# rpng/open_vins

Measured on AMD Instinct MI355X. Metric: MSCKF features/sec per EKF update (30-clone state), higher is better.
Workload: dtype f64; 1 GPU; BASELINE.json configs[2]: 2-camera radtan rig, 30-clone window, 2000 MSCKF features/update, N=248, D=208, online cam extrinsic+intrinsic calib + IMU intrinsics in the state, FEJ; features_total=2000, features_this_rank=2000, clones=30, cameras=2, state_dim=248, measurements_total=100362, parallelism=single GPU

## Files before the change

open_vins_amd/csrc/api_context.inc:

```
using namespace ovg;

static thread_local std::string g_err = "";
static int set_err(int code, const std::string &msg) {
  g_err = msg;
  return code;
}

#define HIPCHK(expr)                                                                                         \
  do {                                                                                                       \
    hipError_t _e = (expr);                                                                                  \
    if (_e != hipSuccess) {                                                                                  \
      return set_err(OVGPU_ERR_HIP, std::string(#expr) + " -> " + hipGetErrorString(_e) + " (" __FILE__ ":" + \
                                        std::to_string(__LINE__) + ")");                                     \
    }                                                                                                        \
  } while (0)

namespace {

template <class T>
struct PinBuf {
  T *p = nullptr;
  size_t cap = 0;
  hipError_t reserve(size_t n) {
    if (n <= cap) return hipSuccess;
// ... 20 lines not shown
    p = nullptr;
    cap = 0;
    hipError_t e = hipMalloc((void **)&p, std::max<size_t>(n, 1) * sizeof(T));
    if (e == hipSuccess) cap = n;
    return e;
  }
  hipError_t grow(size_t n, size_t keep) {
    if (n <= cap) return hipSuccess;
    T *q = nullptr;
    hipError_t e = hipMalloc((void **)&q, n * sizeof(T));
    if (e != hipSuccess) return e;
    if (p && keep > 0) e = hipMemcpy(q, p, std::min(keep, cap) * sizeof(T), hipMemcpyDeviceToDevice);
    if (p) (void)hipFree(p);
    p = q, cap = n;
    return e;
  }
  void release() {
    if (p) (void)hipFree(p);
    p = nullptr;
    cap = 0;
  }
};

struct EventPair {
  hipEvent_t a = nullptr, b = nullptr;
};

}

enum { CTRL_FLAGS = 1, CTRL_ROWS = 2, CTRL_COUNTER = 4, CTRL_PROG0 = 8, CTRL_PROG1 = 16, CTRL_INTS = 64, CHOL_PROG_STRIDE = 24 };

struct LoopComm;
struct UpSeg {
  void *dst;
  uint32_t off, bytes;
};
constexpr int UP_MAX_SEG = 28, UP_BLOCKS = 48;
struct UpBatch {
  UpSeg seg[UP_MAX_SEG];
  int n = 0;
};
__global__ void __launch_bounds__(256) k_upload_scatter(const unsigned char *__restrict__ arena, UpBatch b) {
  const UpSeg sg = b.seg[blockIdx.y];
  const unsigned char *src = arena + sg.off;
  unsigned char *dst = static_cast<unsigned char *>(sg.dst);
  const uint32_t nvec = ((reinterpret_cast<uintptr_t>(dst) & 15) == 0) ? sg.bytes >> 4 : 0;
  typedef unsigned int u32x4 __attribute__((ext_vector_type(4)));
  const u32x4 *s4 = reinterpret_cast<const u32x4 *>(src);
  u32x4 *d4 = reinterpret_cast<u32x4 *>(dst);
  for (uint32_t i = blockIdx.x * 256 + threadIdx.x; i < nvec; i += gridDim.x * 256) d4[i] = __builtin_nontemporal_load(s4 + i);
  for (uint32_t i = (nvec << 4) + blockIdx.x * 256 + threadIdx.x; i < sg.bytes; i += gridDim.x * 256) dst[i] = src[i];
}

struct ovgpu_ctx {
  int device = 0;
  hipStream_t stream = nullptr;
  ovgpu_options opts{};
  DevOptions dopt{};
  int lds_limit = 160 * 1024;
  int num_cu = 256;

  bool have_state = false;
  bool poses_only = false;
  int N = 0, C = 0, K = 0, D = 0, LD = 0;
  DevBuf<double> P, P0, clone_qp, clone_qp0, clone_fej, calib_qp, calib_qp0, intr, intr0;
  DevBuf<uint8_t> fisheye;
  DevBuf<int32_t> clone_cov, calib_cov, intr_cov, clone_col, calib_col, intr_col, col_cov;
  DevBuf<uint8_t> col_kind, col_sub;
  DevBuf<uint16_t> col_var;
  DevBuf<double> tab_clone, tab_cam, tab_cc;
  std::vector<int32_t> h_col_cov;
  struct HVar { int cov, size, kind, index; };
  std::vector<HVar> h_vars;
  std::vector<int32_t> h_clone_cov, h_calib_cov, h_intr_cov;
  DevBuf<double> prop_w, prop_in;
  DevBuf<int32_t> prop_ids;
  int L = 0;
  std::vector<int32_t> h_lm_rep;
  std::vector<int32_t> h_feat_lm;
  std::vector<int32_t> h_feat_rep;
  std::vector<int32_t> h_lm_cov, h_lm_col, h_lm_anchor;
  DevBuf<double> pFej, lm_val, lm_fej;
  DevBuf<int32_t> feat_lm, feat_lmcol, feat_lmcov, feat_anchor, lm_cov, lm_col, lm_anchor, lm_repd, lm_index;
  bool slam_rows = false;
  int trk_max = 0, trk_obs = 0;
  int trk_group_order = OVGPU_GROUPS_REFERENCE;
  std::vector<std::vector<int8_t>> trk_h_cams;
  DevBuf<int8_t> trk_order;
  DevBuf<int32_t> trk_count, trk_cam, trk_slot_in, trk_cam_in, trk_sel, trk_nvalid, trk_flag;
  DevBuf<double> trk_time, trk_clone_times, trk_aux;
  DevBuf<float> trk_uv, trk_uvn, trk_uv_in, trk_uvn_in;
  std::unordered_map<int64_t, int32_t> trk_slot_of;
  std::unordered_map<int64_t, int32_t> retri_slot_of;
  DevBuf<double> retri_sys[2], retri_pos, retri_uvd;
  DevBuf<int32_t> retri_int, marg_idx, seed_anchor;
  DevBuf<double> marg_out, seed_pA;
  DevBuf<float> retri_f;
  int retri_gen = 0;
  std::vector<int32_t> trk_free, trk_h_count;
  std::vector<int64_t> trk_h_id;
  DevBuf<double> Ppad, init_ws, dx_seq;
  DevBuf<int32_t> init_ctr, feat_slot;
  bool init_export = false;
  DevBuf<double> isx_arena, isx_save;
  DevBuf<int32_t> isx_cols;
  std::vector<int32_t> h_isx_cols;

  bool have_feats = false;
  bool tri_readable = false;
  bool given_tri = false;
  bool given_has_anchor = false;
  std::vector<int32_t> h_given_status;
  DevBuf<int32_t> given_status;
  int F = 0, M = 0, m_max = 0;
  int64_t rows_total = 0;
  DevBuf<int32_t> meas_offsets;
  DevBuf<uint16_t> meas_cc;
  DevBuf<float> uv, uvn;
  DevBuf<int64_t> row_off;
  DevBuf<double> pA, pG, chi2, chi2_thr;
  int layout_every_update = 0;
  int inst_cb = 0, inst_D = 0;
  DevBuf<int32_t> anchor_pre;
  DevBuf<int32_t> anchor, status, sys_order;
  DevBuf<double> feat_sigma, feat_mult;
  bool have_feat_sigma = false, have_feat_mult = false;
  DevBuf<double> chi2_table;
  int chi2_table_len = 0;
  std::vector<double> h_chi2_table;
  std::vector<int32_t> h_offsets;
  std::vector<int64_t> h_row_off;

  DevBuf<double> Hbig, gate_ws, Rws, Mt, Aaug, Yaug, dx;
  DevBuf<int32_t> flags;
  int W = 1;
  int64_t rows_per_node = 128;
  DevBuf<QrTreeNode> tree_nodes, tree_nodes2;
  int tree_G2 = 0;
  hipStream_t stream2 = nullptr;
  hipEvent_t ev_rows = nullptr;
  bool gram_il = true;
  bool gram_blocks_only = false;
  bool fuse_chol_inputs = true;
  hipEvent_t ev_fork = nullptr, ev_join = nullptr;
  DevBuf<int32_t> leaf_flags;
  int tree_overlap = -1;
  bool tree_nodes_overlap = false, tree_nodes2_overlap = false;
  DevBuf<int32_t> tree_flags;
  DevBuf<int32_t> tree_err;
  int tree_G = 0;
  bool tree_pipelined = true;
  int compress_gram = 1;
  DevBuf<double> gram_part, gram_G, gram_rho, Yaug2, Lw;
  double prior_pivot_tol = 1e-13;
  int last_route = OVGPU_COMPRESS_GRAM;
  bool whiten = true;
  bool gram_is_whitened = false;
  bool prior_on_side = false;
  int feat_variant = 0;
  int feat_nt_max = 0;
  bool featy_ok = false;
  int featy_skip = 0;
  int featy_grid = 0;
  size_t featy_lds = 0;
  DevBuf<double> fs_tq;
  DevBuf<int32_t> fs_inst;
  DevBuf<double> featyb_ws;
  int featy_big = 0;
  bool no_feat_kernel = false;
  bool raw_enable = true;
  int raw_work_const = 12;
  bool raw_veto = false;
  bool raw_one_region = false;
  bool raw_cols_ok = false;
  bool raw_tables_ok = false;
  int raw_j0 = 0;
  int raw_ncls = 0, raw_ntc[RAW_MAXCLS + 1] = {0}, raw_ld[RAW_MAXCLS + 1] = {0}, raw_rcol[RAW_MAXCLS + 1] = {0};
  int64_t raw_base[RAW_MAXCLS + 1] = {0}, raw_rows[RAW_MAXCLS + 1] = {0};
  std::vector<uint8_t> h_cls_of_clone;
  DevBuf<uint8_t> cls_of_clone;
  DevBuf<int32_t> raw_featbase, raw_dst;
  DevBuf<double> Hraw;
  DevBuf<gram::GramRegionWG> gram_wg;
  int gram_wg_n = 0, gram_wg_tiles = 0;
  gram::GramRegionSum raw_rs;
  bool last_stack_raw = false;
  DevBuf<int32_t> feat_counter, fs_minfo, fs_meas_feat, fs_pos;
  DevBuf<int32_t> fs_slots;
  std::vector<int32_t> h_order;
  std::vector<uint16_t> h_cc;
  DevBuf<double> fs_rows, fs_V, fs_z, fs_w;
  void *comm = nullptr;
  struct LoopComm *loop = nullptr;
  int comm_rank = 0, comm_world = 1;
  DevBuf<double> comm_buf;
  DevBuf<int32_t> chol_prog;
  DevBuf<int32_t> ctrl;
  unsigned ctrl_clean = 0;
  unsigned ctrl_pre = 0;
  DevBuf<double> chol_uinv;
  PinBuf<double> h_tri;
  int chol_slot = 0;
  bool no_chol_pipe = false;
  int tri_waves = 0;
  int feat_shape = 0;
  int feat_nta_max = 0;
  PinBuf<unsigned char> up_arena;
  PinBuf<unsigned char> down_arena;
  size_t up_off = 0, up_want = 8u << 20;
  UpBatch up_batch;
  const unsigned char *up_arena_dev = nullptr;
  bool up_kernel = true;
  UpBatch down_batch;
  unsigned char *down_arena_dev = nullptr;
  const double *chi2_table_dev = nullptr;
  int chi2_table_dev_len = 0;
  bool up_dirty = false;
  bool up_fallback = false;
  bool gram_fp32 = false;
  bool want_stack_f32 = false;
  bool stack_is_f32 = false;
  int stack_ldf = 0;
  DevBuf<float> Hbig32, gram32_part;
  DevBuf<int32_t> gram32_tiles;
  int gram32_ntm = 0, gram32_P = 0;
  int Lw_D = -1;
  DevBuf<long long> dbg_cycles;
  int tsqr_workers = 0;
  bool async_pending = false;
  bool last_update_tform = false;
  bool force_tsqr = false;
  int chol_spin_limit = 1 << 22;
  int chol_timeouts = 0;
  int mode_a_factor = 0;
  bool factor_from_gram = false;
  bool last_factor_from_gram = false;
  bool chol_timed_out = false;
  bool prior_pending = false;
  bool prior_overlap = true;
  const double *last_uinv = nullptr;
  const double *prior_uinv = nullptr;
  int layout_fpw = 8;
  bool unwhiten_blocked = true;
  bool pchol_blocked = true;
  bool speculative_prior = true;
  DevBuf<int32_t> gram_dropped, rows_used;
  int sys_grid = 1;
  int64_t gate_ws_stride = 0;
  bool sys_rows_global = false;
  DevBuf<double> sys_rows_ws;
  int m_lds_max = 0;
  size_t sys_lds_bytes = 0;
  int row_stride = 48;

  std::vector<EventPair> ev_compress, ev_update, ev_system;
  size_t ev_used = 0;
  bool timed_this_update = false;
  bool timing = true;
  int timing_period = 1;
  uint64_t timing_seq = 0;
};

template <class T>
static hipError_t remove_record(DevBuf<T> &a, DevBuf<T> &tmp, int n, int w, int idx, hipStream_t s) {
  const size_t tail = (size_t)(n - idx - 1) * w;
  if (tail == 0) return hipSuccess;
  hipError_t e = tmp.reserve(tail);
  if (e != hipSuccess) return e;
  e = hipMemcpyAsync(tmp.p, a.p + (size_t)(idx + 1) * w, tail * sizeof(T), hipMemcpyDeviceToDevice, s);
  if (e != hipSuccess) return e;
  return hipMemcpyAsync(a.p + (size_t)idx * w, tmp.p, tail * sizeof(T), hipMemcpyDeviceToDevice, s);
}

static hipError_t upload(void *dst, const void *src, size_t bytes, hipStream_t s) {
  if (bytes == 0) return hipSuccess;
  return hipMemcpyAsync(dst, src, bytes, hipMemcpyHostToDevice, s);
}

static hipError_t upload_flush(ovgpu_ctx *c);
static hipError_t upload_begin(ovgpu_ctx *c) {
  if (!c->up_dirty) c->up_off = 0;
  if (c->up_want > c->up_arena.cap) {
    if (c->up_dirty) {
      if (hipError_t ef = upload_flush(c); ef != hipSuccess) return ef;
      hipError_t e = hipStreamSynchronize(c->stream);
      if (e != hipSuccess) return e;
      c->up_dirty = false, c->up_fallback = false, c->up_off = 0;
    }
    if (hipError_t e = c->up_arena.reserve(c->up_want); e != hipSuccess) return e;
    void *dev = nullptr;
    c->up_arena_dev = hipHostGetDevicePointer(&dev, c->up_arena.p, 0) == hipSuccess ? static_cast<const unsigned char *>(dev) : nullptr;
  }
  return hipSuccess;
}
__global__ void __launch_bounds__(256) k_download_gather(unsigned char *__restrict__ arena, UpBatch b) {
  const UpSeg sg = b.seg[blockIdx.y];
  unsigned char *dst = arena + sg.off;
  const unsigned char *src = static_cast<const unsigned char *>(sg.dst);
  const uint32_t nvec = ((reinterpret_cast<uintptr_t>(src) & 15) == 0) ? sg.bytes >> 4 : 0;
  typedef unsigned int u32x4 __attribute__((ext_vector_type(4)));
  const u32x4 *s4 = reinterpret_cast<const u32x4 *>(src);
  u32x4 *d4 = reinterpret_cast<u32x4 *>(dst);
  for (uint32_t i = blockIdx.x * 256 + threadIdx.x; i < nvec; i += gridDim.x * 256) __builtin_nontemporal_store(s4[i], d4 + i);
  for (uint32_t i = (nvec << 4) + blockIdx.x * 256 + threadIdx.x; i < sg.bytes; i += gridDim.x * 256) dst[i] = src[i];
}
static hipError_t down_reserve(ovgpu_ctx *c, size_t bytes) {
// ... 199 lines not shown
```

open_vins_amd/csrc/api_pipeline.inc:

```
static int enqueue_triangulate(ovgpu_ctx *c, const double *seed_pA = nullptr, const int32_t *seed_anchor = nullptr) {
  if (c->F == 0) return OVGPU_OK;
  TriParams p;
  p.seed_pA = seed_pA, p.seed_anchor = seed_anchor, p.anchor_pre = c->anchor_pre.p;
  p.F = c->F, p.C = c->C, p.K = c->K;
  p.meas_offsets = c->meas_offsets.p, p.meas_cc = c->meas_cc.p, p.uvn = c->uvn.p, p.tab_cc = c->tab_cc.p;
  p.p_FinA = c->pA.p, p.p_FinG = c->pG.p, p.anchor_meas = c->anchor.p, p.status = c->status.p;
  p.opt = c->dopt;
  const size_t lds = (size_t)c->K * c->C * 12 * sizeof(double);
  int wpb = c->tri_waves;
  if (wpb == 0) {
    wpb = 4;
    const int room = c->num_cu - 6;
    for (int w = 4; w <= 8 && room > 0; w *= 2) {
      const int blocks = (c->F + w - 1) / w;
      if (blocks <= room) {
        if (4 * blocks >= 3 * room) wpb = w;
        break;
      }
    }
  }
  hipLaunchKernelGGL(k_triangulate, dim3((c->F + wpb - 1) / wpb), dim3(64 * wpb), lds, c->stream, p);
  HIPCHK(hipGetLastError());
  return OVGPU_OK;
}
// ... 392 lines not shown
  double sigma2 = -1.0;
  const int32_t *pred = nullptr;
  double *dx = nullptr;
  bool keep_flags = false;
};

struct CholSource {
  int src = chol::CH_SRC_MATRIX;
  const TformParams *t = nullptr;
};
static int enqueue_chol_carry(ovgpu_ctx *c, const EkfParams &p, hipStream_t s, double *Lt, const CholSource &from = CholSource());

static int enqueue_ekf(ovgpu_ctx *c, const EkfJob &job = EkfJob()) {
  {
    const int rdp = drop_pending_prior(c);
    if (rdp != OVGPU_OK) return rdp;
  }
  c->last_update_tform = false;
  EkfParams p;
  const bool tri = job.R == nullptr;
  p.N = c->N, p.D = tri ? c->D : job.rows, p.DC = c->D, p.LD = c->LD, p.LA = p.D + c->N + 1, p.tri = tri ? 1 : 0, p.pred = job.pred;
  p.R = tri ? c->Rws.p : job.R, p.col_cov = job.col_cov ? job.col_cov : c->col_cov.p, p.P = c->P.p, p.Mt = c->Mt.p, p.A = c->Aaug.p, p.Y = c->Yaug.p;
  p.dx = job.dx ? job.dx : c->dx.p, p.flags = c->flags.p;
  p.sigma2 = job.sigma2 >= 0.0 ? job.sigma2 : c->dopt.sigma_pix_sq;
  hipStream_t s = c->stream;
  if (!job.keep_flags) HIPCHK(ctrl_zero(c, CTRL_FLAGS, c->flags.p, 4 * sizeof(int32_t), s));
  const int tm = (p.D + 15) / 16, tn = (p.N + 15) / 16;
  hipLaunchKernelGGL(k_ekf_mt, dim3((tm * tn + 3) / 4), dim3(256), 0, s, p);
  hipLaunchKernelGGL(k_ekf_s, dim3((tm * tm + 3) / 4), dim3(256), 0, s, p);
  {
    const int rcc = enqueue_chol_carry(c, p, s, nullptr);
    if (rcc != OVGPU_OK) return rcc;
  }
  hipLaunchKernelGGL(k_ekf_dx, dim3((p.N + 255) / 256), dim3(256), 0, s, p);
  hipLaunchKernelGGL(k_ekf_pupdate, dim3((tn * tn + 3) / 4), dim3(256), 0, s, p);
  const int n = std::max(c->C, c->K);
  hipLaunchKernelGGL(k_boxplus, dim3((n + 255) / 256), dim3(256), 0, s, c->C, c->K, p.dx, c->clone_cov.p, c->calib_cov.p, c->intr_cov.p,
                     c->clone_qp.p, c->calib_qp.p, c->intr.p, job.pred);
  HIPCHK(hipGetLastError());
  return launch_build_tables(c);
}

static bool chol_pipe_usable(const ovgpu_ctx *c, int D) { return !c->no_chol_pipe && D <= 16 * chol::CH_TMAX && D >= 1; }
static int enqueue_chol_carry(ovgpu_ctx *c, const EkfParams &p, hipStream_t s, double *Lt, const CholSource &from) {
  if (chol_pipe_usable(c, p.D)) {
    HIPCHK(c->chol_prog.reserve(CHOL_PROG_STRIDE + 16));
    HIPCHK(c->chol_uinv.reserve((size_t)2 * 16 * 256));
    const int slot = (c->chol_slot++) & 1;
    chol::CholParams q;
    q.D = p.D, q.LA = p.LA, q.A = p.A, q.Y = p.Y, q.Lt = Lt, q.flags = p.flags, q.diag0 = p.diag0, q.pivot_tol = p.pivot_tol, q.pred = p.pred;
    q.prog = c->chol_prog.p + CHOL_PROG_STRIDE * slot, q.uinv = c->chol_uinv.p + (size_t)slot * 16 * 256, q.err = p.flags + 2, q.dbg = c->dbg_cycles.p;
    q.spin_limit = c->chol_spin_limit;
    q.n_arrive = chol::chol_tile_waves((p.D + 15) / 16);
    q.src = from.src, q.N = p.N, q.pred_not = p.pred_not;
    if (from.src != chol::CH_SRC_MATRIX) {
      const TformParams &t = *from.t;
      q.col_cov = t.col_cov, q.P = t.P, q.G = t.G, q.LG = t.LG, q.inv_sigma2 = t.inv_sigma2, q.Y1 = t.Y1;
    }
    c->last_uinv = q.uinv;
    HIPCHK(ctrl_zero(c, slot ? CTRL_PROG1 : CTRL_PROG0, q.prog, 16 * sizeof(int32_t), s));
    const int carried = (p.LA - p.D + 15) / 16;
    static bool attr_f2 = false;
    if (!attr_f2) {
      (void)hipFuncSetAttribute((const void *)chol::k_chol_fused, hipFuncAttributeMaxDynamicSharedMemorySize, (int)chol::chol_lds_bytes());
      attr_f2 = true;
    }
    hipLaunchKernelGGL(chol::k_chol_fused, dim3(1 + (carried + chol::CH_FC - 1) / chol::CH_FC), dim3(64 * (chol::CH_FW + 1)), chol::chol_lds_bytes(), s, q);
    HIPCHK(hipGetLastError());
    return OVGPU_OK;
  }
  if (from.src != chol::CH_SRC_MATRIX) return set_err(OVGPU_ERR_INVALID, "the step-wise factorisation needs its work matrix assembled");
  const int TM = (p.D + 15) / 16, TL = (p.LA + 15) / 16;
  for (int kb = 0; kb < p.D; kb += 16) {
    const int tb = kb / 16;
    int jobs = TL - tb;
    for (int it = tb + 1; it < TM; it++) jobs += TL - it;
    hipLaunchKernelGGL(k_ekf_chol_step, dim3((jobs + 3) / 4), dim3(256), 0, s, p, kb);
  }
  if (Lt) {
    TformParams t;
    t.D = p.D, t.LA = p.LA, t.Y1 = p.Y, t.Lw = Lt;
    hipLaunchKernelGGL(k_tf_lt, dim3((unsigned)((p.D * p.D + 255) / 256)), dim3(256), 0, s, t);
  }
  HIPCHK(hipGetLastError());
  return OVGPU_OK;
}

static int enqueue_ekf_gram(ovgpu_ctx *c, int part, bool side = false) {
  const int D = c->D, N = c->N, LA = D + N + 1;
  HIPCHK(c->Yaug2.reserve((size_t)D * LA));
  HIPCHK(c->gram_rho.reserve(std::max(N, D)));
  HIPCHK(c->Lw.reserve((size_t)D * (D + 8)));
  if (c->Lw_D != D) {
    HIPCHK(hipMemsetAsync(c->Lw.p, 0, sizeof(double) * D * (D + 8), c->stream));
    c->Lw_D = D;
  }
  EkfParams p;
  p.N = N, p.D = D, p.DC = D, p.LD = c->LD, p.LA = LA, p.tri = 1, p.pred = nullptr;
  p.R = nullptr, p.col_cov = c->col_cov.p, p.P = c->P.p, p.Mt = c->Mt.p, p.A = c->Aaug.p, p.Y = c->Yaug.p;
  p.dx = c->dx.p, p.flags = c->flags.p, p.sigma2 = c->dopt.sigma_pix_sq;
  TformParams t;
  t.N = N, t.D = D, t.LA = LA, t.LG = 16 * ((c->LD + 15) / 16), t.col_cov = c->col_cov.p, t.G = c->gram_G.p, t.P = c->P.p;
  t.A = c->Aaug.p, t.Y1 = c->Yaug.p, t.W = c->Mt.p, t.inv_sigma2 = 1.0 / c->dopt.sigma_pix_sq, t.go = c->flags.p + 3, t.diag0 = c->gram_rho.p;
  t.whitened = c->gram_is_whitened ? 1 : 0, t.Lw = c->Lw.p;
  hipStream_t s = c->stream;
  const int tm = (D + 15) / 16, tn = (N + 15) / 16;
  int rc = OVGPU_OK;
  if (part & 1) {
    if (c->prior_on_side) HIPCHK(hipStreamWaitEvent(s, c->ev_join, 0));
    HIPCHK(ctrl_zero(c, CTRL_FLAGS, c->flags.p, 4 * sizeof(int32_t), s));
    hipStream_t sp = s;
    c->prior_on_side = false;
    if (side && part == 1) {
      HIPCHK(hipEventRecord(c->ev_fork, s));
      HIPCHK(hipStreamWaitEvent(c->stream2, c->ev_fork, 0));
      sp = c->stream2;
      c->prior_on_side = true;
    }
    const int64_t elems = (int64_t)D * LA;
    const bool at_source = c->fuse_chol_inputs && chol_pipe_usable(c, D);
    if (!at_source) hipLaunchKernelGGL(k_tf_gather, dim3((unsigned)((elems + 255) / 256)), dim3(256), 0, sp, t);
    p.diag0 = c->gram_rho.p, p.pivot_tol = c->prior_pivot_tol;
    CholSource from;
    if (at_source) from.src = chol::CH_SRC_PRIOR, from.t = &t;
    c->last_uinv = nullptr;
    if ((rc = enqueue_chol_carry(c, p, sp, c->Lw.p, from)) != OVGPU_OK) return rc;
    c->prior_uinv = c->last_uinv;
    p.diag0 = nullptr;
    if (c->prior_on_side) HIPCHK(hipEventRecord(c->ev_join, sp));
    c->prior_pending = true;
  }
  if (part & 2) {
    if (c->prior_on_side) HIPCHK(hipStreamWaitEvent(s, c->ev_join, 0));
    c->prior_pending = false, c->prior_on_side = false;
    p.pred = c->flags.p + 3;
    CholSource from;
    if (t.whitened && c->fuse_chol_inputs && chol_pipe_usable(c, D)) {
      from.src = chol::CH_SRC_WHITENED, from.t = &t;
      p.pred = nullptr, p.pred_not = c->flags.p;
    } else if (t.whitened) {
      hipLaunchKernelGGL(k_tf_abh, dim3((D + 3) / 4), dim3(256), 0, s, t, (const int32_t *)c->flags.p, c->flags.p + 3);
    } else {
      hipLaunchKernelGGL(k_tf_go, dim3(1), dim3(1), 0, s, (const int32_t *)c->flags.p, c->flags.p + 3);
      hipLaunchKernelGGL(k_tf_w, dim3((tm * tm + 3) / 4), dim3(256), 0, s, t);
      hipLaunchKernelGGL(k_tf_t, dim3((tm * tm + 3) / 4), dim3(256), 0, s, t);
      hipLaunchKernelGGL(k_tf_bh, dim3((D + 3) / 4), dim3(256), 0, s, t);
    }
    p.Y = c->Yaug2.p;
    if ((rc = enqueue_chol_carry(c, p, s, nullptr, from)) != OVGPU_OK) return rc;
    TailTables tt;
    tt.C = c->C, tt.K = c->K, tt.clone_cov = c->clone_cov.p, tt.calib_cov = c->calib_cov.p, tt.intr_cov = c->intr_cov.p;
    tt.clone_qp = c->clone_qp.p, tt.calib_qp = c->calib_qp.p, tt.intr = c->intr.p, tt.clone_fej = c->clone_fej.p;
    tt.tab_clone = c->tab_clone.p, tt.tab_cam = c->tab_cam.p, tt.tab_cc = c->tab_cc.p;
    const int nb = (tn * tn + 3) / 4;
    hipLaunchKernelGGL(k_tf_tail, dim3(nb + 1), dim3(256), 0, s, p, (const double *)c->Yaug.p, tt, nb);
    HIPCHK(hipGetLastError());
    c->last_update_tform = true;
    return OVGPU_OK;
  }
  return OVGPU_OK;
}

static int enqueue_speculative_prior(ovgpu_ctx *c) {
  if (!c->speculative_prior || c->prior_pending || !c->have_state || c->poses_only || c->D < 1) return OVGPU_OK;
  if (!(c->stream2 && c->ev_fork && c->ev_join && c->prior_overlap)) return OVGPU_OK;
  if (c->compress_gram != 1 || (c->D + 1 + 15) / 16 > gram::GR_NT_BLK || !c->whiten || !chol_pipe_usable(c, c->D)) return OVGPU_OK;
  const int rc = enqueue_ekf_gram(c, 1, true);
  if (rc != OVGPU_OK) return rc;
  if (c->prior_pending && c->ctrl.p) {
    const int next = c->chol_slot & 1;
    int32_t *lo = next ? c->rows_used.p : c->chol_prog.p;
    const size_t n = next ? (size_t)(8 + 16) : (size_t)(16 + 3);
    HIPCHK(hipMemsetAsync(lo, 0, n * sizeof(int32_t), c->stream));
    c->ctrl_pre = CTRL_ROWS | CTRL_COUNTER | (next ? CTRL_PROG1 : CTRL_PROG0);
  }
  return OVGPU_OK;
}

static EventPair *next_events(ovgpu_ctx *c, std::vector<EventPair> &v, size_t idx) {
  if (idx >= v.size()) {
    if (v.size() >= 8192) return nullptr;
    v.resize(idx + 1);
  }
  EventPair &e = v[idx];
  if (!e.a) {
    if (hipEventCreate(&e.a) != hipSuccess || hipEventCreate(&e.b) != hipSuccess) return nullptr;
  }
  return &e;
}

enum { STAGE_LOCAL = 1, STAGE_EKF = 2 };

static int enqueue_pipeline_body(ovgpu_ctx *c, int stages, bool slam, bool factor_stays, bool gram_only);
static int enqueue_pipeline(ovgpu_ctx *c, int stages, bool slam = false, bool factor_stays = false, bool gram_only = false) {
  c->ctrl_clean = 0;
  if (c->have_state && !c->prior_on_side && !c->prior_pending && c->ctrl.p) {
    HIPCHK(hipSetDevice(c->device));
    HIPCHK(hipMemsetAsync(c->ctrl.p, 0, CTRL_INTS * sizeof(int32_t), c->stream));
    c->ctrl_clean = CTRL_FLAGS | CTRL_ROWS | CTRL_COUNTER | CTRL_PROG0 | CTRL_PROG1;
    c->ctrl_pre = 0;
  }
  const int rc = enqueue_pipeline_body(c, stages, slam, factor_stays, gram_only);
  c->ctrl_clean = 0;
  return rc;
}
static int enqueue_pipeline_body(ovgpu_ctx *c, int stages, bool slam, bool factor_stays, bool gram_only) {
  if (!c->have_state || c->poses_only) return set_err(OVGPU_ERR_NO_STATE, "ovgpu_set_state was never called");
  if (!c->have_feats) return set_err(OVGPU_ERR_NO_STATE, "ovgpu_set_features was never called (or the state changed since)");
  HIPCHK(hipSetDevice(c->device));
  if (c->slam_rows != slam) {
    const int rcl = set_row_layout(c, slam);
    if (rcl != OVGPU_OK) return rcl;
  }
  EventPair *eu = nullptr, *ec = nullptr, *es = nullptr;
  bool tform = false;
  if (c->timing && (c->timing_period <= 1 || c->timing_seq++ % c->timing_period == 0)) {
    eu = next_events(c, c->ev_update, c->ev_used);
    ec = next_events(c, c->ev_compress, c->ev_used);
    es = next_events(c, c->ev_system, c->ev_used);
    if (eu && ec && es) c->ev_used++;
    else eu = ec = es = nullptr;
  }
  c->timed_this_update = eu != nullptr;
  if (eu) HIPCHK(hipEventRecord(eu->a, c->stream));
  int rc = OVGPU_OK;
  const bool fits = (c->LD + 15) / 16 <= gram::GR_NT_BLK && c->F > 0;
  tform = !gram_only && c->compress_gram == 1 && !c->force_tsqr && fits && (stages & STAGE_EKF) != 0 && (stages & STAGE_LOCAL) != 0;
  const bool factor_gram = c->factor_from_gram && !gram_only && c->mode_a_factor != 0 && !c->force_tsqr && c->F > 0 && (c->LD + 15) / 16 <= gram::GR_NT_BLK &&
                           (stages & STAGE_EKF) == 0 && (stages & STAGE_LOCAL) != 0 && c->whiten && !c->gram_fp32 && !slam;
  c->factor_from_gram = false, c->last_factor_from_gram = factor_gram;
  c->force_tsqr = false;
  const bool need_prior = (tform || factor_gram || (gram_only && fits)) && (stages & STAGE_LOCAL) != 0;
  const bool whiten = need_prior && c->whiten;
  const bool side = need_prior && c->stream2 != nullptr && c->ev_fork != nullptr && c->ev_join != nullptr && c->prior_overlap;
  if (need_prior && !c->prior_pending && (rc = enqueue_ekf_gram(c, 1, side)) != OVGPU_OK) return rc;
  if (!need_prior && c->prior_pending && (rc = drop_pending_prior(c)) != OVGPU_OK) return rc;
  if (c->layout_every_update) {
    const int rct = enqueue_batch_tables(c, true);
    if (rct != OVGPU_OK) return rct;
  }
  if (stages & STAGE_LOCAL) {
    if (c->given_tri) {
      if (c->F > 0) HIPCHK(hipMemcpyAsync(c->status.p, c->given_status.p, sizeof(int32_t) * c->F, hipMemcpyDeviceToDevice, c->stream));
    } else if ((rc = enqueue_triangulate(c)) != OVGPU_OK) return rc;
    if (es) HIPCHK(hipEventRecord(es->a, c->stream));
    c->want_stack_f32 = c->gram_fp32 && whiten && (gram_only || tform) && (c->LD + 31) / 32 <= 12;
    c->raw_veto = factor_gram;
    rc = enqueue_system(c, -1, 0, whiten);
    c->want_stack_f32 = false, c->raw_veto = false;
    if (rc != OVGPU_OK) return rc;
    if (es) HIPCHK(hipEventRecord(es->b, c->stream));
    if (need_prior) c->gram_is_whitened = whiten;
    if (ec) HIPCHK(hipEventRecord(ec->a, c->stream));
    if (gram_only || tform) {
      if ((c->LD + 15) / 16 > gram::GR_NT_BLK) return set_err(OVGPU_ERR_CAPACITY, "the Gram route holds at most 383 Jacobian columns");
      rc = enqueue_compress_gram(c, false);
    } else if (factor_gram) {
      rc = enqueue_compress_gram(c, true);
      if (rc == OVGPU_OK) {
        if (c->prior_on_side) HIPCHK(hipStreamWaitEvent(c->stream, c->ev_join, 0));
        c->prior_pending = false, c->prior_on_side = false;
        if ((c->D + 15) / 16 <= 16 && c->unwhiten_blocked && c->prior_uinv)
          hipLaunchKernelGGL(k_unwhiten_blk<16>, dim3((c->D + 15) / 16), dim3(256), 0, c->stream, c->D, c->LD, c->Rws.p, (const double *)c->Yaug.p, c->D + c->N + 1,
                             c->prior_uinv, (const int32_t *)nullptr, (const int32_t *)c->flags.p);
        else if ((c->D + 15) / 16 <= 16)
          hipLaunchKernelGGL(k_unwhiten<16>, dim3((c->D + 15) / 16), dim3(64), 0, c->stream, c->D, c->LD, c->Rws.p, (const double *)c->Yaug.p, c->D + c->N + 1,
                             (const int32_t *)nullptr, (const int32_t *)c->flags.p);
        else
          hipLaunchKernelGGL(k_unwhiten<24>, dim3((c->D + 15) / 16), dim3(64), 0, c->stream, c->D, c->LD, c->Rws.p, (const double *)c->Yaug.p, c->D + c->N + 1,
                             (const int32_t *)nullptr, (const int32_t *)c->flags.p);
        HIPCHK(hipGetLastError());
      }
    } else {
      rc = enqueue_compress(c);
    }
    if (rc != OVGPU_OK) return rc;
    if (ec) HIPCHK(hipEventRecord(ec->b, c->stream));
  }
  if (stages & STAGE_EKF) {
    if ((rc = tform ? enqueue_ekf_gram(c, 2) : enqueue_ekf(c)) != OVGPU_OK) return rc;
    c->last_route = tform ? OVGPU_COMPRESS_GRAM : OVGPU_COMPRESS_TSQR;
  }
  if (eu) HIPCHK(hipEventRecord(eu->b, c->stream));
  return OVGPU_OK;
}

struct PendingFeatOut {
  bool active = false;
  int32_t *feat_status = nullptr;
  double *chi2 = nullptr, *chi2_thresh = nullptr, *p_FinG = nullptr;
  ovgpu_update_stats *stats = nullptr;
  size_t o_st = 0, o_c2 = 0, o_th = 0, o_pg = 0, o_gb = 0, end = 0;
};
static void unpack_feature_outputs(ovgpu_ctx *c, const PendingFeatOut &q) {
  const int F = c->F;
  int32_t *feat_status = q.feat_status;
  double *chi2 = q.chi2, *chi2_thresh = q.chi2_thresh, *p_FinG = q.p_FinG;
  ovgpu_update_stats *stats = q.stats;
  std::vector<int32_t> st(F);
  if (F > 0) {
    const unsigned char *h = c->down_arena.p;
    std::memcpy(st.data(), h + q.o_st, sizeof(int32_t) * F);
    if (chi2) std::memcpy(chi2, h + q.o_c2, sizeof(double) * F);
    if (chi2_thresh) std::memcpy(chi2_thresh, h + q.o_th, sizeof(double) * F);
    if (p_FinG) std::memcpy(p_FinG, h + q.o_pg, sizeof(double) * 3 * F);
    if (stats) std::memcpy(&stats->n_gate_bound, h + q.o_gb, sizeof(int32_t));
  }
  const double qnan = std::nan("");
// ... 293 lines not shown
```

open_vins_amd/csrc/api_state.inc:

```

const char *ovgpu_last_error(void) { return g_err.c_str(); }

void ovgpu_default_options(ovgpu_options *o) {
  if (!o) return;
  std::memset(o, 0, sizeof(*o));
  o->chi2_multipler = 5.0, o->sigma_pix = 1.0;
  o->triangulate_1d = 0, o->refine_features = 1, o->max_runs = 5;
  o->init_lamda = 1e-3, o->max_lamda = 1e10, o->min_dx = 1e-6, o->min_dcost = 1e-6, o->lam_mult = 10;
  o->min_dist = 0.10, o->max_dist = 60, o->max_baseline = 40, o->max_cond_number = 10000;
  o->do_fej = 1, o->do_calib_camera_pose = 1, o->do_calib_camera_intrinsics = 1;
  o->feat_rep_msckf = OVGPU_REP_GLOBAL_3D;
}

double ovgpu_chi2_quantile_95(int dof) { return chi2_quantile_95(dof); }
int ovgpu_abi_version(void) { return OVGPU_ABI_VERSION; }

int ovgpu_create(const ovgpu_options *opts, int device, ovgpu_ctx **out) {
  if (!opts || !out) return set_err(OVGPU_ERR_INVALID, "null argument");
  *out = nullptr;
  int ndev = 0;
  hipError_t e = hipGetDeviceCount(&ndev);
  if (e != hipSuccess || ndev <= 0)
    return set_err(OVGPU_ERR_NO_DEVICE, std::string("no HIP device (") + hipGetErrorString(e) + "): this library has no CPU fallback");
  if (device < 0 || device >= ndev) return set_err(OVGPU_ERR_INVALID, "device index out of range");
  if (opts->feat_rep_msckf < 0 || opts->feat_rep_msckf > OVGPU_REP_ANCHORED_INVERSE_DEPTH_SINGLE)
    return set_err(OVGPU_ERR_INVALID, "unknown feature representation");
  HIPCHK(hipSetDevice(device));
  ovgpu_ctx *c = new ovgpu_ctx();
  c->device = device;
  c->opts = *opts;
  hipDeviceProp_t prop;
  HIPCHK(hipGetDeviceProperties(&prop, device));
  c->num_cu = prop.multiProcessorCount > 0 ? prop.multiProcessorCount : 256;
  c->lds_limit = (int)std::min<size_t>(prop.sharedMemPerBlock, 160 * 1024);
  HIPCHK(hipStreamCreateWithFlags(&c->stream, hipStreamNonBlocking));
  HIPCHK(c->ctrl.reserve(CTRL_INTS));
  HIPCHK(hipMemset(c->ctrl.p, 0, CTRL_INTS * sizeof(int32_t)));
  c->flags.p = c->ctrl.p, c->flags.cap = 4;
  c->rows_used.p = c->ctrl.p + 24, c->rows_used.cap = 2;
  c->feat_counter.p = c->ctrl.p + 26, c->feat_counter.cap = 1;
  c->chol_prog.p = c->ctrl.p + 8, c->chol_prog.cap = 40;
  c->ctrl_pre = 0;
  DevOptions &d = c->dopt;
  d.chi2_multipler = opts->chi2_multipler;
  d.sigma_pix_sq = opts->sigma_pix * opts->sigma_pix;
  d.init_lamda = opts->init_lamda, d.max_lamda = opts->max_lamda, d.min_dx = opts->min_dx, d.min_dcost = opts->min_dcost;
  d.lam_mult = opts->lam_mult, d.min_dist = opts->min_dist, d.max_dist = opts->max_dist, d.max_baseline = opts->max_baseline;
  d.max_cond_number = opts->max_cond_number;
  d.triangulate_1d = opts->triangulate_1d, d.refine_features = opts->refine_features, d.max_runs = opts->max_runs;
  d.do_fej = opts->do_fej, d.do_calib_pose = opts->do_calib_camera_pose, d.do_calib_intr = opts->do_calib_camera_intrinsics;
  d.feat_rep = opts->feat_rep_msckf;
  d.gate_always_factor = opts->gate_always_factor != 0;
  if (d.feat_rep == OVGPU_REP_ANCHORED_INVERSE_DEPTH_SINGLE) d.feat_rep = OVGPU_REP_ANCHORED_MSCKF_INVERSE_DEPTH;
  c->row_stride = (d.feat_rep >= OVGPU_REP_ANCHORED_3D) ? 72 : 48;
  if (opts->compress_route < 0 || opts->compress_route > OVGPU_COMPRESS_PCHOLQR || opts->compress_route == 2  || opts->tsqr_overlap < 0 || opts->tsqr_overlap > 2 || opts->tsqr_workers < 0) {
    ovgpu_destroy(c);
    return set_err(OVGPU_ERR_INVALID, "bad library switch in ovgpu_options");
  }
  c->tree_pipelined = opts->tsqr_no_pipeline == 0;
  c->prior_overlap = opts->no_prior_overlap == 0;
  c->compress_gram = opts->compress_route == OVGPU_COMPRESS_TSQR ? 0 : 1;
  c->mode_a_factor = opts->compress_route == OVGPU_COMPRESS_TSQR ? 0 : 2;
  c->tree_overlap = opts->tsqr_overlap == 0 ? -1 : (opts->tsqr_overlap == 1 ? 1 : 0);
  c->whiten = opts->gram_no_whiten == 0;
  c->prior_pivot_tol = opts->prior_pivot_tol > 0.0 ? opts->prior_pivot_tol : 1e-13;
  c->tsqr_workers = opts->tsqr_workers;
  c->no_feat_kernel = opts->no_fast_feature_kernel != 0;
  c->no_chol_pipe = opts->no_single_launch_cholesky != 0;
  c->feat_shape = opts->feature_kernel_shape;
  c->gram_fp32 = opts->gram_fp32 != 0;
  if (hipEventCreateWithFlags(&c->ev_rows, hipEventDisableTiming) != hipSuccess) c->no_feat_kernel = true;
  int prio_lo = 0, prio_hi = 0;
  (void)hipDeviceGetStreamPriorityRange(&prio_lo, &prio_hi);
  if (hipStreamCreateWithPriority(&c->stream2, hipStreamNonBlocking, prio_hi) != hipSuccess || hipEventCreateWithFlags(&c->ev_fork, hipEventDisableTiming) != hipSuccess ||
      hipEventCreateWithFlags(&c->ev_join, hipEventDisableTiming) != hipSuccess)
    c->tree_overlap = 0;
  (void)hipFuncSetAttribute((const void *)k_system_t<false>, hipFuncAttributeMaxDynamicSharedMemorySize, c->lds_limit);
  (void)hipFuncSetAttribute((const void *)k_system_t<true>, hipFuncAttributeMaxDynamicSharedMemorySize, c->lds_limit);
  (void)hipFuncSetAttribute((const void *)k_triangulate, hipFuncAttributeMaxDynamicSharedMemorySize, c->lds_limit);
  c->timing = opts->no_timing == 0;
  *out = c;
  return OVGPU_OK;
}

void ovgpu_destroy(ovgpu_ctx *c) {
  if (!c) return;
  (void)hipSetDevice(c->device);
  (void)upload_sync(c, c->stream);
  if (c->stream2) (void)hipStreamSynchronize(c->stream2);
  for (auto &e : c->ev_compress) {
    if (e.a) (void)hipEventDestroy(e.a);
    if (e.b) (void)hipEventDestroy(e.b);
  }
  for (auto &e : c->ev_update) {
    if (e.a) (void)hipEventDestroy(e.a);
    if (e.b) (void)hipEventDestroy(e.b);
  }
  for (auto &e : c->ev_system) {
    if (e.a) (void)hipEventDestroy(e.a);
    if (e.b) (void)hipEventDestroy(e.b);
  }
  c->P.release(), c->P0.release(), c->clone_qp.release(), c->clone_qp0.release(), c->clone_fej.release();
  c->calib_qp.release(), c->calib_qp0.release(), c->intr.release(), c->intr0.release(), c->fisheye.release();
  c->clone_cov.release(), c->calib_cov.release(), c->intr_cov.release(), c->clone_col.release(), c->calib_col.release();
  c->intr_col.release(), c->col_cov.release(), c->col_kind.release(), c->col_sub.release(), c->col_var.release();
  c->tab_clone.release(), c->tab_cam.release(), c->tab_cc.release();
  c->retri_sys[0].release(), c->retri_sys[1].release(), c->retri_pos.release(), c->retri_uvd.release(), c->retri_int.release(), c->retri_f.release(), c->marg_idx.release(), c->marg_out.release(), c->seed_anchor.release(), c->seed_pA.release();
  c->meas_offsets.release(), c->meas_cc.release(), c->uv.release(), c->uvn.release(), c->row_off.release();
  c->pA.release(), c->pG.release(), c->chi2.release(), c->chi2_thr.release(), c->anchor.release(), c->anchor_pre.release(), c->status.release(), c->sys_order.release(), c->feat_sigma.release(), c->feat_mult.release();
  c->Hbig32.release(), c->gram32_part.release(), c->gram32_tiles.release();
  c->up_arena.release(), c->down_arena.release();
  c->chi2_table.release(), c->Hbig.release(), c->gate_ws.release(), c->Rws.release(), c->tree_nodes.release(), c->tree_nodes2.release(), c->tree_flags.release(), c->tree_err.release(), c->Mt.release(), c->Aaug.release(), c->Yaug.release();
  c->pFej.release(), c->lm_val.release(), c->lm_fej.release(), c->feat_lm.release(), c->feat_lmcol.release(), c->feat_lmcov.release(), c->lm_cov.release();
  c->feat_anchor.release(), c->lm_col.release(), c->lm_anchor.release(), c->lm_index.release(), c->Ppad.release(), c->init_ws.release(), c->dx_seq.release();
  c->init_ctr.release(), c->feat_slot.release(), c->prop_w.release(), c->prop_in.release(), c->prop_ids.release();
  c->trk_count.release(), c->trk_cam.release(), c->trk_slot_in.release(), c->trk_cam_in.release(), c->trk_sel.release(), c->trk_nvalid.release(), c->trk_flag.release();
  c->trk_time.release(), c->trk_clone_times.release(), c->trk_aux.release(), c->trk_uv.release(), c->trk_uvn.release(), c->trk_uv_in.release(), c->trk_uvn_in.release();
  c->dx.release(), c->given_status.release();
  c->flags.p = nullptr, c->rows_used.p = nullptr, c->feat_counter.p = nullptr, c->chol_prog.p = nullptr;
  c->ctrl.release();
  c->gram_part.release(), c->gram_G.release(), c->gram_rho.release(), c->Yaug2.release(), c->gram_dropped.release(), c->Lw.release(), c->dbg_cycles.release();
  c->chol_uinv.release();
  c->h_tri.release();
  c->fs_slots.release(), c->fs_minfo.release(), c->fs_meas_feat.release(), c->fs_pos.release(), c->fs_rows.release(), c->fs_V.release(), c->fs_z.release(), c->fs_w.release(), c->fs_tq.release(), c->fs_inst.release(), c->featyb_ws.release();
  if (c->ev_fork) (void)hipEventDestroy(c->ev_fork);
  if (c->ev_join) (void)hipEventDestroy(c->ev_join);
  if (c->stream2) (void)hipStreamDestroy(c->stream2);
  c->comm_buf.release();
  if (c->ev_rows) (void)hipEventDestroy(c->ev_rows);
  c->leaf_flags.release();
  if (c->stream) (void)hipStreamDestroy(c->stream);
  delete c;
}

static int lm_dof(int rep) { return rep == OVGPU_REP_ANCHORED_INVERSE_DEPTH_SINGLE ? 1 : 3; }
static bool lm_any_anchored(const ovgpu_ctx *c) {
  for (int l = 0; l < c->L; l++)
    if (c->h_lm_rep[l] >= OVGPU_REP_ANCHORED_3D) return true;
  return false;
}
static int lm_uniform_dof(const ovgpu_ctx *c) {
  int d = c->L > 0 ? lm_dof(c->h_lm_rep[0]) : 3;
  for (int l = 1; l < c->L; l++)
    if (lm_dof(c->h_lm_rep[l]) != d) return 0;
  return d;
}

static hipError_t ctrl_zero(ovgpu_ctx *c, unsigned bit, void *ptr, size_t bytes, hipStream_t s) {
  if (c->ctrl_clean & bit) {
    c->ctrl_clean &= ~bit;
    c->ctrl_pre &= ~bit;
    return hipSuccess;
  }
  if (c->ctrl_pre & bit) {
    c->ctrl_pre &= ~bit;
    return hipSuccess;
  }
  return hipMemsetAsync(ptr, 0, bytes, s);
}

static int launch_build_tables(ovgpu_ctx *c) {
  const int n = std::max(c->K * c->C, std::max(c->C, c->K));
  hipLaunchKernelGGL(k_build_tables, dim3((n + 255) / 256), dim3(256), 0, c->stream, c->C, c->K, c->clone_qp.p, c->clone_fej.p, c->calib_qp.p,
                     c->tab_clone.p, c->tab_cam.p, c->tab_cc.p);
  HIPCHK(hipGetLastError());
  return OVGPU_OK;
}

static int build_columns(ovgpu_ctx *c, bool defer_flush = false) {
  std::vector<ovgpu_ctx::HVar> vars = c->h_vars;
  for (int l = 0; l < c->L; l++) vars.push_back({c->h_lm_cov[l], lm_dof(c->h_lm_rep[l]), COL_LANDMARK, l});
  std::stable_sort(vars.begin(), vars.end(), [](const ovgpu_ctx::HVar &a, const ovgpu_ctx::HVar &b) { return a.cov < b.cov; });
  const int C = c->C, K = c->K, N = c->N;
  std::vector<int32_t> clone_col(C, -1), calib_col(K, -1), intr_col(K, -1), col_cov;
  std::vector<uint8_t> col_kind, col_sub;
  std::vector<uint16_t> col_var;
  c->h_lm_col.assign(c->L, -1);
  int D = 0;
  for (const auto &v : vars) {
    if (v.cov < 0 || v.cov + v.size > N) return set_err(OVGPU_ERR_INVALID, "covariance id out of range");
    if (v.kind == COL_CLONE) clone_col[v.index] = D;
    if (v.kind == COL_CALIB_POSE) calib_col[v.index] = D;
    if (v.kind == COL_CALIB_INTR) intr_col[v.index] = D;
    if (v.kind == COL_LANDMARK) c->h_lm_col[v.index] = D;
    for (int i = 0; i < v.size; i++) {
      col_cov.push_back(v.cov + i);
      col_kind.push_back((uint8_t)v.kind);
      col_var.push_back((uint16_t)v.index);
      col_sub.push_back((uint8_t)((v.kind == COL_LANDMARK && v.size == 1) ? 2 : i));
    }
    D += v.size;
  }
  if (D + 1 > 512) return set_err(OVGPU_ERR_CAPACITY, "more than 511 Jacobian columns");
  c->D = D, c->LD = D + 1;
  {
    c->raw_cols_ok = false, c->raw_ncls = 0, c->raw_tables_ok = false;
    int calib_end = 0, clone_min = D;
    for (int k = 0; k < K; k++) calib_end = std::max(calib_end, std::max(calib_col[k] >= 0 ? calib_col[k] + 6 : 0, intr_col[k] >= 0 ? intr_col[k] + 8 : 0));
    for (int i = 0; i < C; i++)
      if (clone_col[i] >= 0) clone_min = std::min(clone_min, clone_col[i]);
    const int NTf = (D + 1 + 15) / 16;
    if (c->L == 0 && calib_end <= clone_min && NTf >= 6 && NTf <= 15) {
      const int top = NTf == 15 ? 15 : ((NTf + 1) & ~1);
      int n = 0;
      for (int t = 4; t < top && n < RAW_MAXCLS - 1 && !c->raw_one_region; t += 2)
        if (16 * t - 4 >= calib_end + 6) c->raw_ntc[n] = t, c->raw_ld[n] = 16 * t - 3, c->raw_rcol[n] = 16 * t - 4, n++;
      c->raw_ntc[n] = top, c->raw_ld[n] = D + 1, c->raw_rcol[n] = D, n++;
      c->raw_ncls = n;
      c->raw_ntc[RAW_NEG] = top, c->raw_ld[RAW_NEG] = D + 1, c->raw_rcol[RAW_NEG] = D;
      c->h_cls_of_clone.assign(C, (uint8_t)(n - 1));
      for (int i = 0; i < C; i++) {
        int k = 0;
        while (k < n - 1 && clone_col[i] + 6 > c->raw_rcol[k]) k++;
        c->h_cls_of_clone[i] = (uint8_t)k;
      }
      HIPCHK(c->cls_of_clone.reserve(C));
      HIPCHK(upload_deferred(c, c->cls_of_clone.p, c->h_cls_of_clone.data(), C));
      c->raw_j0 = clone_min + 6;
      c->raw_cols_ok = true;
    }
  }
  c->h_col_cov = col_cov;
  HIPCHK(c->col_cov.reserve(D));
  HIPCHK(c->col_kind.reserve(D));
  HIPCHK(c->col_sub.reserve(D));
  HIPCHK(c->col_var.reserve(D));
  HIPCHK(c->Mt.reserve((size_t)D * N));
  HIPCHK(c->Aaug.reserve((size_t)D * (D + N + 1)));
  HIPCHK(c->Yaug.reserve((size_t)D * (D + N + 1)));
  hipStream_t s = c->stream;
  (void)s;
  HIPCHK(upload_deferred(c, c->clone_col.p, clone_col.data(), sizeof(int32_t) * C));
  HIPCHK(upload_deferred(c, c->calib_col.p, calib_col.data(), sizeof(int32_t) * K));
  HIPCHK(upload_deferred(c, c->intr_col.p, intr_col.data(), sizeof(int32_t) * K));
  HIPCHK(upload_deferred(c, c->col_cov.p, col_cov.data(), sizeof(int32_t) * D));
  HIPCHK(upload_deferred(c, c->col_kind.p, col_kind.data(), D));
  HIPCHK(upload_deferred(c, c->col_sub.p, col_sub.data(), D));
  HIPCHK(upload_deferred(c, c->col_var.p, col_var.data(), sizeof(uint16_t) * D));
  if (c->L > 0) HIPCHK(upload_deferred(c, c->lm_col.p, c->h_lm_col.data(), sizeof(int32_t) * c->L));
  if (!defer_flush) HIPCHK(upload_fence(c, c->stream));
  c->have_feats = false;
  c->tri_readable = false;
  return OVGPU_OK;
}

int ovgpu_set_state(ovgpu_ctx *c, const ovgpu_state_view *st) {
  if (!c || !st) return set_err(OVGPU_ERR_INVALID, "null argument");
  { const int rdp = drop_pending_prior(c); if (rdp != OVGPU_OK) return rdp; }
  if (st->N <= 0 || st->C <= 0 || st->K <= 0) return set_err(OVGPU_ERR_INVALID, "empty state");
  if (st->C > OVG_MAX_CLONES || st->K > OVG_MAX_CAMS) return set_err(OVGPU_ERR_CAPACITY, "too many clones / cameras");
  if (!st->P || !st->clone_q_p || !st->clone_q_p_fej || !st->clone_cov_id || !st->calib_q_p || !st->intrinsics || !st->cam_is_fisheye ||
      !st->calib_cov_id || !st->intr_cov_id)
    return set_err(OVGPU_ERR_INVALID, "null state array");
  HIPCHK(hipSetDevice(c->device));
  HIPCHK(upload_begin(c));
  const int N = st->N, C = st->C, K = st->K;

  c->h_vars.clear();
  for (int k = 0; k < K; k++) {
    if (c->dopt.do_calib_pose && st->calib_cov_id[k] >= 0) c->h_vars.push_back({st->calib_cov_id[k], 6, COL_CALIB_POSE, k});
    if (c->dopt.do_calib_intr && st->intr_cov_id[k] >= 0) c->h_vars.push_back({st->intr_cov_id[k], 8, COL_CALIB_INTR, k});
  }
  for (int i = 0; i < C; i++) c->h_vars.push_back({st->clone_cov_id[i], 6, COL_CLONE, i});
  c->N = N, c->C = C, c->K = K;
  c->L = 0, c->h_lm_rep.clear(), c->h_lm_cov.clear(), c->h_lm_col.clear(), c->h_lm_anchor.clear();
  c->row_stride = (c->dopt.feat_rep >= OVGPU_REP_ANCHORED_3D) ? 72 : 48;
  HIPCHK(c->clone_col.reserve(C));
  HIPCHK(c->calib_col.reserve(K));
  HIPCHK(c->intr_col.reserve(K));
  {
    const int rcb = build_columns(c, true);
    if (rcb != OVGPU_OK) return rcb;
  }
  const int D = c->D;

// ... 422 lines not shown
```

open_vins_amd/csrc/k_tail.h:

```cpp
#pragma once
#include "k_ekf.h"
#include "k_triangulate.h"

namespace ovg {

struct TailTables {
  int C, K;
  const int32_t *clone_cov, *calib_cov, *intr_cov;
  double *clone_qp, *calib_qp, *intr;
  const double *clone_fej;
  double *tab_clone, *tab_cam, *tab_cc;
};
__global__ void __launch_bounds__(256) k_tf_tail(EkfParams p, const double *Y1, TailTables t, int nb) {
  if ((int)blockIdx.x < nb) {
    tf_pupdate_tile(p, Y1, blockIdx.x * 4 + (threadIdx.x >> 6), threadIdx.x & 63);
    return;
  }
  for (int i = threadIdx.x; i < p.N; i += 256) ekf_dx_item(p, i);
  __syncthreads();
  const int n1 = t.C > t.K ? t.C : t.K;
  if (!ekf_skipped(p))
    for (int i = threadIdx.x; i < n1; i += 256) boxplus_item(i, t.C, t.K, p.dx, t.clone_cov, t.calib_cov, t.intr_cov, t.clone_qp, t.calib_qp, t.intr);
  __syncthreads();
  const int n2 = t.K * t.C > n1 ? t.K * t.C : n1;
  for (int i = threadIdx.x; i < n2; i += 256) build_tables_item(i, t.C, t.K, t.clone_qp, t.clone_fej, t.calib_qp, t.tab_clone, t.tab_cam, t.tab_cc);
}


struct RestoreParams {
  int N2, nC, nK7, nK8, C, K;
  double *P, *clone_qp, *calib_qp, *intr;
  const double *P0, *clone_qp0, *calib_qp0, *intr0, *clone_fej;
  double *tab_clone, *tab_cam, *tab_cc;
};
__global__ void __launch_bounds__(256) k_restore_state(RestoreParams r) {
  const int i = blockIdx.x * 256 + threadIdx.x;
  if (i < r.N2) r.P[i] = r.P0[i];
  if (i < r.nC) r.clone_qp[i] = r.clone_qp0[i];
  if (i < r.nK7) r.calib_qp[i] = r.calib_qp0[i];
  if (i < r.nK8) r.intr[i] = r.intr0[i];
  const int nt = r.K * r.C > (r.C > r.K ? r.C : r.K) ? r.K * r.C : (r.C > r.K ? r.C : r.K);
  if (i < nt) build_tables_item(i, r.C, r.K, r.clone_qp0, r.clone_fej, r.calib_qp0, r.tab_clone, r.tab_cam, r.tab_cc);
}

}
```

Measured before the change: 2.866 million features/s.

## Split EKF dx reduction across blocks with last-block-done partial sum

The state correction dx was previously computed by a single block looping over all D rows per state entry, which serialised a long dot product on one CU. The new tail kernel spreads the D rows across ceil(D/16) chunk blocks. Each block writes partial sums to a scratch buffer, and an atomic counter picks the last block to finish. That block sums the partials, writes dx, and then runs boxplus and table rebuilding as before. This adds a workspace, an atomic counter reset by the last block, and threadfence-based ordering, and it changes the floating-point summation order.

```diff
diff --git a/open_vins_amd/csrc/api_context.inc b/open_vins_amd/csrc/api_context.inc
--- a/open_vins_amd/csrc/api_context.inc
+++ b/open_vins_amd/csrc/api_context.inc
@@ -196,6 +196,8 @@
   bool tree_pipelined = true;
   int compress_gram = 1;
   DevBuf<double> gram_part, gram_G, gram_rho, Yaug2, Lw;
+  DevBuf<double> tail_dx_part;
+  DevBuf<int32_t> tail_dx_cnt;
   double prior_pivot_tol = 1e-13;
   int last_route = OVGPU_COMPRESS_GRAM;
   bool whiten = true;
diff --git a/open_vins_amd/csrc/api_pipeline.inc b/open_vins_amd/csrc/api_pipeline.inc
--- a/open_vins_amd/csrc/api_pipeline.inc
+++ b/open_vins_amd/csrc/api_pipeline.inc
@@ -568,8 +568,14 @@
     tt.C = c->C, tt.K = c->K, tt.clone_cov = c->clone_cov.p, tt.calib_cov = c->calib_cov.p, tt.intr_cov = c->intr_cov.p;
     tt.clone_qp = c->clone_qp.p, tt.calib_qp = c->calib_qp.p, tt.intr = c->intr.p, tt.clone_fej = c->clone_fej.p;
     tt.tab_clone = c->tab_clone.p, tt.tab_cam = c->tab_cam.p, tt.tab_cc = c->tab_cc.p;
-    const int nb = (tn * tn + 3) / 4;
-    hipLaunchKernelGGL(k_tf_tail, dim3(nb + 1), dim3(256), 0, s, p, (const double *)c->Yaug.p, tt, nb);
+    const int nb = (tn * tn + 3) / 4, nch = tail_dx_chunks(D);
+    HIPCHK(c->tail_dx_part.reserve((size_t)nch * N));
+    if (!c->tail_dx_cnt.p) {
+      HIPCHK(c->tail_dx_cnt.reserve(1));
+      HIPCHK(hipMemsetAsync(c->tail_dx_cnt.p, 0, sizeof(int32_t), s));
+    }
+    tt.dx_part = c->tail_dx_part.p, tt.dx_cnt = c->tail_dx_cnt.p;
+    hipLaunchKernelGGL(k_tf_tail, dim3(nch + nb), dim3(256), 0, s, p, (const double *)c->Yaug.p, tt);
     HIPCHK(hipGetLastError());
     c->last_update_tform = true;
     return OVGPU_OK;
diff --git a/open_vins_amd/csrc/api_state.inc b/open_vins_amd/csrc/api_state.inc
--- a/open_vins_amd/csrc/api_state.inc
+++ b/open_vins_amd/csrc/api_state.inc
@@ -120,7 +120,7 @@
   c->flags.p = nullptr, c->rows_used.p = nullptr, c->feat_counter.p = nullptr, c->chol_prog.p = nullptr;
   c->ctrl.release();
   c->gram_part.release(), c->gram_G.release(), c->gram_rho.release(), c->Yaug2.release(), c->gram_dropped.release(), c->Lw.release(), c->dbg_cycles.release();
-  c->chol_uinv.release();
+  c->chol_uinv.release(), c->tail_dx_part.release(), c->tail_dx_cnt.release();
   c->h_tri.release();
   c->fs_slots.release(), c->fs_minfo.release(), c->fs_meas_feat.release(), c->fs_pos.release(), c->fs_rows.release(), c->fs_V.release(), c->fs_z.release(), c->fs_w.release(), c->fs_tq.release(), c->fs_inst.release(), c->featyb_ws.release();
   if (c->ev_fork) (void)hipEventDestroy(c->ev_fork);
diff --git a/open_vins_amd/csrc/k_tail.h b/open_vins_amd/csrc/k_tail.h
--- a/open_vins_amd/csrc/k_tail.h
+++ b/open_vins_amd/csrc/k_tail.h
@@ -10,16 +10,61 @@
   double *clone_qp, *calib_qp, *intr;
   const double *clone_fej;
   double *tab_clone, *tab_cam, *tab_cc;
+  double *dx_part;
+  int32_t *dx_cnt;
 };
-__global__ void __launch_bounds__(256) k_tf_tail(EkfParams p, const double *Y1, TailTables t, int nb) {
-  if ((int)blockIdx.x < nb) {
-    tf_pupdate_tile(p, Y1, blockIdx.x * 4 + (threadIdx.x >> 6), threadIdx.x & 63);
+constexpr int TL_DX_ROWS = 16;
+__host__ __device__ inline int tail_dx_chunks(int D) { return (D + TL_DX_ROWS - 1) / TL_DX_ROWS; }
+
+__device__ __forceinline__ double ekf_dx_chunk(const EkfParams &p, int ch, int i) {
+  const double *Y = p.Y + p.D + i, *y = p.Y + p.D + p.N;
+  const int r0 = TL_DX_ROWS * ch;
+  double a[TL_DX_ROWS], b[TL_DX_ROWS];
+#pragma unroll
+  for (int j = 0; j < TL_DX_ROWS; j++) {
+    const size_t off = (size_t)min(r0 + j, p.D - 1) * p.LA;
+    a[j] = Y[off], b[j] = y[off];
+  }
+  double s[4] = {0.0, 0.0, 0.0, 0.0};
+#pragma unroll
+  for (int j = 0; j < TL_DX_ROWS; j++) s[j & 3] = fma(r0 + j < p.D ? a[j] : 0.0, b[j], s[j & 3]);
+  return (s[0] + s[1]) + (s[2] + s[3]);
+}
+
+__global__ void __launch_bounds__(256) k_tf_tail(EkfParams p, const double *Y1, TailTables t) {
+  const int nch = tail_dx_chunks(p.D);
+  if ((int)blockIdx.x >= nch) {
+    tf_pupdate_tile(p, Y1, ((int)blockIdx.x - nch) * 4 + (threadIdx.x >> 6), threadIdx.x & 63);
     return;
   }
-  for (int i = threadIdx.x; i < p.N; i += 256) ekf_dx_item(p, i);
+  __shared__ int is_last;
+  const bool skipped = ekf_skipped(p);
+  if (!skipped)
+    for (int i = threadIdx.x; i < p.N; i += 256) t.dx_part[(size_t)blockIdx.x * p.N + i] = ekf_dx_chunk(p, blockIdx.x, i);
+  __threadfence();
+  __syncthreads();
+  if (threadIdx.x == 0) is_last = atomicAdd(t.dx_cnt, 1) == nch - 1;
+  __syncthreads();
+  if (!is_last) return;
+  __threadfence();
+  if (threadIdx.x == 0) *t.dx_cnt = 0;
+  for (int i = threadIdx.x; i < p.N; i += 256) {
+    double v = 0.0;
+    if (!skipped) {
+      for (int c0 = 0; c0 < nch; c0 += 16) {
+        double q[16];
+#pragma unroll
+        for (int c = 0; c < 16; c++) q[c] = t.dx_part[(size_t)min(c0 + c, nch - 1) * p.N + i];
+#pragma unroll
+        for (int c = 0; c < 16; c++)
+          if (c0 + c < nch) v += q[c];
+      }
+    }
+    p.dx[i] = v;
+  }
   __syncthreads();
   const int n1 = t.C > t.K ? t.C : t.K;
-  if (!ekf_skipped(p))
+  if (!skipped)
     for (int i = threadIdx.x; i < n1; i += 256) boxplus_item(i, t.C, t.K, p.dx, t.clone_cov, t.calib_cov, t.intr_cov, t.clone_qp, t.calib_qp, t.intr);
   __syncthreads();
   const int n2 = t.K * t.C > n1 ? t.K * t.C : n1;
```

New measurement: 2.887 million features/s (median of 6 runs). Within noise of the previous version (+0.7%).
